# hherlyng/knp-emi-cgx

Measured on AMD Instinct MI355X. Metric: MDoF/s per implicit timestep (assembly+GMRES), higher is better.
Workload: dtype f64

## Files before the change

### knp-emi-cgx_amd/csrc/knp_internal.hpp

```cpp
#pragma once
#include <hip/hip_runtime.h>

#include <cstdint>
#include <string>
#include <vector>

#include "knpemi_hip.h"

#define KNP_NPROF 5

struct KnpHostGraph {
    int dim = 0, nv1 = 0;
    int n_v = 0, n_v_owned = 0, n_c = 0, n_c_owned = 0, n_g = 0, n_q = 0;
    int n_nodes = 0, n_nodes_owned = 0;
    std::vector<int32_t> node_i, node_e;
    std::vector<int32_t> node_vertex;
    std::vector<uint8_t> node_side;
    std::vector<int32_t> pair_ptr;
    std::vector<int32_t> pair_col;
    std::vector<int32_t> pair_row;
    std::vector<double> pair_M, pair_K;
    std::vector<int32_t> contrib_ptr;
    std::vector<int32_t> contrib_cell;
    std::vector<double> contrib_k;
// ... 163 lines not shown
    int l0_upload = 0;
    int32_t *at0_rp = nullptr, *at0_ci = nullptr;
    double* at0_v = nullptr;
    float* at0_vf = nullptr;
    int at0_lanes = 8;
    double *pt = nullptr, *pt_phi = nullptr;
    float *pt_f = nullptr, *pt_phi_f = nullptr;
};

struct KnpSidePrep {
    enum Kind { NONE, LEFT_ENQUEUED, LEFT_DEFERRED, LEFT_CONCURRENT, FLEX } kind = NONE;
    const double* b = nullptr;
    bool fused = false;
    bool left() const { return kind != NONE && kind != FLEX; }
};

struct knp_ctx {
    std::string err;
    hipStream_t stream = nullptr;
    int device = 0;
    KnpHostGraph g;
    double dt = 0, F = 1, C_M = 1, psi = 1;
    int n_ions = 3;
    double z[KNP_MAX_IONS] = {1, 1, -1}, Di[KNP_MAX_IONS] = {1, 1, 1}, De[KNP_MAX_IONS] = {1, 1, 1};
    int64_t nnz = 0, n_pairs = 0, n_contrib = 0, n_gp = 0, n_gc = 0;
    int n_dof_owned = 0, n_dof_local = 0;
    int32_t* d_cells = nullptr;
    uint8_t* d_cell_side = nullptr;
    double* d_coords = nullptr;
    int32_t* d_node_vertex = nullptr;
    uint8_t* d_node_side = nullptr;
    int32_t *d_node_i = nullptr, *d_node_e = nullptr;
    int32_t *d_pair_ptr = nullptr, *d_pair_col = nullptr, *d_pair_row = nullptr;
    double *d_pair_M = nullptr, *d_pair_K = nullptr;
    double2* d_pair_MK = nullptr;
    int32_t *d_contrib_ptr = nullptr, *d_contrib_cell = nullptr;
    double* d_contrib_k = nullptr;
    int32_t *d_node_cell_ptr = nullptr, *d_node_cell = nullptr;
    uint8_t* d_contrib_slot = nullptr;
    int64_t* d_tc_meta = nullptr;
    double* d_tc_k = nullptr;
    uint8_t* d_tc_slot = nullptr;
    int64_t n_tc = 0;
    int asm_stage = 0;
    int asm_dmax = 0;
    int64_t n_node_cells = 0;
    uint8_t* d_ncv = nullptr;
    double* d_knod = nullptr;
    int32_t* d_fv = nullptr;
    double* d_fmeas = nullptr;
    int32_t* d_gamma_prog = nullptr;
    double *d_qp = nullptr, *d_qw = nullptr;
    int32_t *d_gv_vertex = nullptr, *d_gv_node_i = nullptr, *d_gv_node_e = nullptr, *d_node_gv = nullptr;
    int32_t *d_gptr = nullptr, *d_gcol = nullptr, *d_grow = nullptr, *d_gq_i = nullptr, *d_gq_e = nullptr,
            *d_gdiag = nullptr;
    int32_t *d_gcptr = nullptr, *d_gc_facet = nullptr, *d_gc_lab = nullptr;
    double *d_at = nullptr, *d_ac = nullptr, *d_ax = nullptr;
    int32_t *d_gx_i = nullptr, *d_gx_e = nullptr;
    double* d_p_vals = nullptr;
    double* d_px = nullptr;
    int pc_coupled_phi = 0;
    bool have_A = false, have_P = false, have_cc = false;
    double* d_cbar = nullptr;
    double* d_fmat = nullptr;
    double* d_fvec = nullptr;
    std::vector<KnpProgram> progs;
    int32_t** d_prog_code = nullptr;
    double** d_prog_consts = nullptr;
    int32_t* d_prog_len = nullptr;
    int32_t* d_prog_nconsts = nullptr;
    int prog_regs = 0, prog_len_cap = 0, prog_consts_cap = 0;
    size_t gamma_lds_set = 0;
    void* jit_module = nullptr;
    void* jit_fn[3] = {nullptr, nullptr, nullptr};
    std::string jit_msg;
    bool progs_dirty = true;
    int max_prog = -1;
    const double* src_i[KNP_MAX_IONS] = {nullptr, nullptr, nullptr};
    const double* src_e[KNP_MAX_IONS] = {nullptr, nullptr, nullptr};
    bool have_sources = false;
    int pc_kind = KNP_PC_NONE;
    int fused_dots = 1;
    int spmv_dots = 1;
    double* d_vbj = nullptr;
    KnpAmgHier hier[KNP_MAX_HIER];
    int amg_fp32 = 0;
    float* d_p_vals_f = nullptr;
    double* d_ML = nullptr;
    double* d_cc = nullptr;
    double *d_t2 = nullptr, *d_w2 = nullptr;
    int ns_on = 0;
    int spmv_group = 8;
    int pc_group = 8;
    int asm_group = 8;
    int gm_restart = 0;
    double* d_V = nullptr;
    double *d_w = nullptr, *d_t = nullptr;
    double* d_Z = nullptr;
    int z_cap = 0;
    double* d_partial = nullptr;
    double* d_red = nullptr;
    double* h_red = nullptr;
    double* h_red_dev = nullptr;
    double* mirror() const { return (allreduce && p2p_red < 0) ? nullptr : h_red_dev; }
    int64_t phi_count_cached = -1;
    int64_t* h_seq = nullptr;
    int64_t* h_seq_dev = nullptr;
    int64_t seq_counter = 0;
    int asm_full = 0;
    double asm_dt = -1.0;
    int n_bc = 0;
    int32_t* d_bc_dofs = nullptr;
    int defl_m = 0;
    int32_t* d_defl_mode = nullptr;
    double* d_defl_einv = nullptr;
    double* d_y = nullptr;
    double* d_gm = nullptr;
    int gm_cap = 0;
    int64_t n_norm_fallback = 0;
    int n_red_blocks = 0;
    knp_halo_fn halo = nullptr;
    knp_allreduce_fn allreduce = nullptr;
    knp_level_comm_fn level_comm = nullptr;
    void* comm_user = nullptr;
    KnpP2P* p2p = nullptr;
    int p2p_fine = -1;
    int p2p_red = -1;
    bool hook_allreduce() const { return allreduce && p2p_red < 0; }
    int comm_rc = 0;
    int n_int = 0, n_bnd = 0;
    int32_t *d_nodes_int = nullptr, *d_nodes_bnd = nullptr;
    hipStream_t stream3 = nullptr;
    hipEvent_t ev_x = nullptr, ev_halo = nullptr;
    hipStream_t stream2 = nullptr;
    hipEvent_t ev_fork = nullptr, ev_join = nullptr;
    KnpSidePrep prep;
    bool side_ws = false;
    double *d_t2_s = nullptr, *d_w2_s = nullptr, *d_wb = nullptr, *d_partial_s = nullptr;
    hipStream_t stream_asm = nullptr;
    hipEvent_t ev_fork_asm = nullptr, ev_asm = nullptr;
    bool asm_pending = false;
    double last_bnorm = 0.0;
    int64_t n_allreduce = 0, n_halo = 0, n_readback = 0;
    int64_t n_fused_dots = 0;
    int64_t n_spmv_dots = 0;
    std::vector<hipEvent_t> tm_events;
    size_t tm_used = 0;
    KnpDiagMap diag_cells, diag_facets;
    KnpDiagMap diag_flux;
    double2* d_flux_rec = nullptr;
    KnpDiagMap diag_phim;
    int32_t* diag_code = nullptr;
    int diag_n_instr = 0, diag_n_regs = 0, diag_n_consts = 0;
    double diag_consts[KNP_DIAG_MAX_CONSTS] = {};
    bool diag_prog = false;
    KnpEmi emi;
    int prof_on = 0;
    std::vector<hipEvent_t> prof_pool;
    struct ProfRec { hipEvent_t a, b; int cls; };
    std::vector<ProfRec> prof_recs;
    double prof_ms[KNP_NPROF] = {0, 0, 0, 0, 0};
    int64_t prof_n[KNP_NPROF] = {0, 0, 0, 0, 0};
};

int knp_host_threads();
```

### knp-emi-cgx_amd/csrc/knp_kernels.hip

```cpp
#include <hip/hip_runtime.h>
#include <hip/hip_ext.h>

#include <algorithm>
#include <cmath>
#include <cstdio>
#include <cstdlib>
#include <cstring>
#include <new>

#include "knp_internal.hpp"

#define HIPCHK(call)                                                                       \
    do {                                                                                   \
        hipError_t e_ = (call);                                                            \
        if (e_ != hipSuccess) {                                                            \
            ctx->err = std::string(#call) + ": " + hipGetErrorString(e_);                  \
            return KNP_E_HIP;                                                              \
        }                                                                                  \
    } while (0)
#define KCHK(expr)                         \
    do {                                   \
        int rc_ = (expr);                  \
        if (rc_ != KNP_OK) return rc_;     \
    } while (0)
// ... 4163 lines not shown
            else launch_restrict_first_t<double>(st, L.R_lanes, nc, L.R_rp, Rci, L.R_v, L.r, C.b, cc, C.inv_diag, C.d, C.x);
            launch_spmv_mp<1>(st, C.A_lanes, C.n, C.A_rp, C.A_ci, C.A_v, C.A_vf, C.x, C.b, C.r);
        }
    }
    for (int l = H.cfused ? 0 : nl - 2; l >= 0; --l) {
        KnpAmgLevel& L = H.lv[l];
        KnpAmgLevel& C = H.lv[l + 1];
        const double c = cheb_c(L);
        const int n_act = L.S_n_act > 0 ? L.S_n_act : L.S_rows;
        const int32_t* rp = L.S_n_act > 0 ? L.S_act_rp : L.S_rp;
        if (l > 0) {
            if (L.S_vf) launch_level_up_t<float, 0>(st, L.S_lanes, n_act, L.S_n_act > 0 ? L.S_act_rows : nullptr, rp, L.S_ci, L.S_vf, C.x, L.inv_diag, L.b, L.r, L.x, c, c, L.x, nullptr);
            else launch_level_up_t<double, 0>(st, L.S_lanes, n_act, L.S_n_act > 0 ? L.S_act_rows : nullptr, rp, L.S_ci, L.S_v, C.x, L.inv_diag, L.b, L.r, L.x, c, c, L.x, nullptr);
        } else if (phi) {
            const int32_t* rows = L.S_n_act > 0 ? L.S_act_rows_c : nullptr;
            const double* ccp = ctx->pc_kind == KNP_PC_AMG_LT ? nullptr : ctx->d_cc;
            if (L.S_vf) launch_level_up_t<float, 1>(st, L.S_lanes, L.S_n_act > 0 ? n_act : nn, rows, rp, L.S_ci, L.S_vf, C.x, L.dinv_c, b, L.r, nullptr, c, c, z, ccp);
            else launch_level_up_t<double, 1>(st, L.S_lanes, L.S_n_act > 0 ? n_act : nn, rows, rp, L.S_ci, L.S_v, C.x, L.dinv_c, b, L.r, nullptr, c, c, z, ccp);
        } else {
            if (L.S_vf) launch_level_up_t<float, 0>(st, L.S_lanes, n_act, L.S_n_act > 0 ? L.S_act_rows : nullptr, rp, L.S_ci, L.S_vf, C.x, L.inv_diag, b, L.r, nullptr, c, c, z, nullptr);
            else launch_level_up_t<double, 0>(st, L.S_lanes, n_act, L.S_n_act > 0 ? L.S_act_rows : nullptr, rp, L.S_ci, L.S_v, C.x, L.inv_diag, b, L.r, nullptr, c, c, z, nullptr);
        }
    }
}

static int check_hier(knp_ctx* ctx, int h) {
    KnpAmgHier& H = ctx->hier[h];
    if (H.levels < 1 || H.lv[0].n != ctx->n_dof_owned) { ctx->err = "AMG hierarchy " + std::to_string(h) + " not supplied"; return KNP_E_STATE; }
    if (H.native0 == 0 && H.lv[0].A_nnz == 0 && H.levels > 1) {
        ctx->err = "AMG hierarchy " + std::to_string(h) + ": level 0 has no operator (uploaded for knp_amg_use_native_level0, which is off)";
        return KNP_E_STATE;
    }
    for (int l = 0; l < H.levels - 1; ++l) {
        const int expect = H.lv[l].repl_n > 0 ? H.lv[l + 1].n : H.lv[l + 1].n_loc;
        if (H.lv[l].n_coarse != expect) { ctx->err = "AMG level sizes inconsistent"; return KNP_E_STATE; }
        if (H.lv[l].repl_n > 0 && H.lv[l].repl_n != H.lv[l + 1].n) { ctx->err = "replicated coarse size mismatch"; return KNP_E_STATE; }
    }
    if (H.nc > 0 && H.nc != H.lv[H.levels - 1].n) { ctx->err = "AMG coarse inverse size mismatch"; return KNP_E_STATE; }
    return KNP_OK;
}

static int build_level_scaled(knp_ctx* ctx, int hidx, int l) {
    KnpAmgLevel& L = ctx->hier[hidx].lv[l];
    const double c = 1.0 / (0.5 * (1.1 + 0.1) * L.lambda_max);
    double* dloc = nullptr;
    HIPCHK(hipMalloc((void**)&dloc, (size_t)std::max(L.n_loc, 1) * sizeof(double)));
    HIPCHK(hipMemsetAsync(dloc, 0, (size_t)std::max(L.n_loc, 1) * sizeof(double), ctx->stream));
    HIPCHK(hipMemcpyAsync(dloc, L.inv_diag, (size_t)L.n * sizeof(double), hipMemcpyDeviceToDevice, ctx->stream));
    if (L.dist && level_comm_on(ctx)) level_exchange(ctx, hidx, l, 0, dloc);
    const int nblk = (int)std::min<int64_t>(nblocks(L.A_nnz), 8192);
    if (L.A_vf) {
        HIPCHK(hipMalloc((void**)&L.At_vf, (size_t)L.A_nnz * sizeof(float)));
        hipLaunchKernelGGL((k_build_at<float, float>), dim3(nblk), dim3(NT), 0, ctx->stream, L.A_nnz, L.A_ci, L.A_vf, dloc, c, L.At_vf);
    } else {
        HIPCHK(hipMalloc((void**)&L.At_v, (size_t)L.A_nnz * sizeof(double)));
        hipLaunchKernelGGL((k_build_at<double, double>), dim3(nblk), dim3(NT), 0, ctx->stream, L.A_nnz, L.A_ci, L.A_v, dloc, c, L.At_v);
    }
    HIPCHK(hipGetLastError());
    HIPCHK(hipStreamSynchronize(ctx->stream));
    (void)hipFree(dloc);
    if (ctx->comm_rc != KNP_OK) { const int rc = ctx->comm_rc; ctx->comm_rc = KNP_OK; return rc; }
    return KNP_OK;
}

int knp_pc_setup(knp_ctx* ctx, int32_t kind) {
    CHECK_CTX(ctx);
    side_discard(ctx);
    KCHK(join_asm(ctx));
    if (kind != KNP_PC_NONE && kind != KNP_PC_VBJACOBI && kind != KNP_PC_AMG && kind != KNP_PC_AMG_BT && kind != KNP_PC_AMG_LT) { ctx->err = "unknown pc kind"; return KNP_E_ARG; }
    if (kind == KNP_PC_AMG) KCHK(check_hier(ctx, 0));
    if (kind == KNP_PC_AMG_BT || kind == KNP_PC_AMG_LT) {
        KCHK(check_hier(ctx, 0));
        KCHK(check_hier(ctx, 1));
        if (!ctx->d_t2) {
            HIPCHK(hipMalloc((void**)&ctx->d_t2, std::max(ctx->n_dof_local, 1) * sizeof(double)));
            HIPCHK(hipMalloc((void**)&ctx->d_w2, std::max(ctx->n_dof_local, 1) * sizeof(double)));
            HIPCHK(hipMemset(ctx->d_t2, 0, std::max(ctx->n_dof_local, 1) * sizeof(double)));
            HIPCHK(hipMemset(ctx->d_w2, 0, std::max(ctx->n_dof_local, 1) * sizeof(double)));
        }
    }
    ctx->pc_kind = kind;
    ctx->fused_dots = !(getenv("KNP_FUSED_DOTS") && atoi(getenv("KNP_FUSED_DOTS")) == 0);
    ctx->spmv_dots = !(getenv("KNP_SPMV_DOTS") && atoi(getenv("KNP_SPMV_DOTS")) == 0);
    for (int h = 0; h < KNP_MAX_HIER; ++h) ctx->hier[h].fused = 0;
    if (kind == KNP_PC_AMG) ctx->hier[0].fused = fused_eligible(ctx, ctx->hier[0]) ? 1 : 0;
    if (kind == KNP_PC_AMG_BT || kind == KNP_PC_AMG_LT) {
        const bool ok = fused_eligible(ctx, ctx->hier[0]) && fused_eligible(ctx, ctx->hier[1]) && ctx->hier[1].native0 == 3 && ctx->hier[0].native0 == 2 &&
                        ctx->hier[1].lv[0].S_n_act > 0 && ctx->hier[1].lv[0].S_act_rows_c && ctx->hier[1].lv[0].R_ci_c;
        ctx->hier[0].fused = ctx->hier[1].fused = ok ? 1 : 0;
        if (!ok && ctx->hier[1].l0_upload) ctx->hier[1].native0 = 0;
    }
    for (int h = 0; h < KNP_MAX_HIER; ++h) {
        KnpAmgHier& H = ctx->hier[h];
        const bool off = getenv("KNP_BLOCKED") && atoi(getenv("KNP_BLOCKED")) == 0;
        bool ok = !off && H.fused && H.node_nf > 0 && (H.native0 == 1 || H.native0 == 2) && (H.native0 == 1) == (H.node_nf == 4);
        for (int l = 0; ok && l < H.levels - 1; ++l) {
            const KnpAmgLevel& L = H.lv[l];
            ok = L.bR.rp && L.bS.rp && (l == 0 || L.bA.rp) && L.bR.n_rows * H.node_nf == L.n_coarse &&
                 L.bS.n_rows * (l == 0 ? 4 : H.node_nf) == L.n;
        }
        H.blocked = ok ? 1 : 0;
        const bool coff = getenv("KNP_COARSE_FUSED") && atoi(getenv("KNP_COARSE_FUSED")) == 0;
        bool cok = !coff && H.fused && H.levels >= 3;
        for (int l = 1; cok && l < H.levels - 1; ++l) {
            const KnpAmgLevel& L = H.lv[l];
            cok = L.Rt_rp && L.U_rp && (!H.blocked || (L.bRt.rp && L.bU.rp && L.bRt.n_rows * H.node_nf == L.n_coarse && L.bU.n_rows * H.node_nf == L.n));
        }
        H.cfused = cok ? 1 : 0;
        for (int l = 1; cok && l < H.levels - 1; ++l) {
            KnpAmgLevel& L = H.lv[l];
            if (L.cat) continue;
            const size_t nc = (size_t)L.n + (size_t)L.n_coarse;
            HIPCHK(hipMalloc((void**)&L.cat, nc * sizeof(double)));
            HIPCHK(hipMemsetAsync(L.cat, 0, nc * sizeof(double), ctx->stream));
            ctx->side_ws = false;
        }
    }
    for (int h = 0; h < KNP_MAX_HIER; ++h) {
        KnpAmgHier& H = ctx->hier[h];
        const bool off = getenv("KNP_FUSED") && atoi(getenv("KNP_FUSED")) == 0;
        const KnpAmgLevel& L0 = H.lv[0];
        const bool have_pt = H.native0 == 3 ? (H.pt_phi || H.pt_phi_f) : (H.pt || H.pt_f);
        H.l0_fused = (!off && !H.fused && H.native0 > 0 && H.levels >= 2 && H.cheby == 1 && H.pre == 1 && H.post == 1 && L0.S_rp &&
                      L0.S_rows == L0.n && have_pt) ? 1 : 0;
        const bool used = (kind == KNP_PC_AMG && h == 0) || ((kind == KNP_PC_AMG_BT || kind == KNP_PC_AMG_LT) && h < 2);
        double veto[KNP_MAX_AMG_LEVELS] = {0};
        const bool lvl_off = getenv("KNP_FUSED_LEVELS") && atoi(getenv("KNP_FUSED_LEVELS")) == 0;
        for (int l = 1; l < H.levels - 1; ++l) {
            KnpAmgLevel& L = H.lv[l];
            dev_free(L.At_v); dev_free(L.At_vf);
            L.lfused = 0;
            const bool empty_here = L.dist && L.n == 0;
            const bool local_ok = !(!L.S_rp || L.S_rows != L.n || L.S_n_act > 0 || L.n_coarse <= 0 || L.A_nnz <= 0 || !L.inv_diag);
            veto[l] = (!used || off || lvl_off || H.fused || H.cheby != 1 || H.pre != 1 || H.post != 1 || !(local_ok || empty_here)) ? 1.0 : 0.0;
        }
        if (used && H.levels > 2) KCHK(global_sum_small(ctx, veto + 1, H.levels - 2));
        for (int l = 1; l < H.levels - 1; ++l) {
            if (veto[l] != 0.0) continue;
            KCHK(build_level_scaled(ctx, h, l));
            H.lv[l].lfused = 1;
        }
    }
    if (kind == KNP_PC_VBJACOBI && ctx->have_A) {
        const KnpHostGraph& g = ctx->g;
        hipLaunchKernelGGL(k_vbj_extract, dim3(nblocks(g.n_nodes_owned)), dim3(NT), 0, ctx->stream, g.n_nodes_owned,
                           ctx->d_pair_ptr, ctx->d_pair_col, ctx->d_ac, ctx->d_at, ctx->d_ax, ctx->d_node_gv, ctx->d_node_side,
                           ctx->d_gdiag, ctx->d_vbj);
        HIPCHK(hipGetLastError());
    }
    return KNP_OK;
}

__global__ void __launch_bounds__(NT) k_bc_copy(int n_bc, const int32_t* __restrict__ bc_dofs, const double* __restrict__ src,
                                                double* __restrict__ dst, int phi_only) {
    const int i = blockIdx.x * NT + threadIdx.x;
    if (i >= n_bc) return;
    const int d = bc_dofs[i];
    if (phi_only == 2) {
        if ((d & 3) == 3) dst[d >> 2] = src[d];
    } else if (!phi_only || (d & 3) == 3) {
        dst[d] = src[d];
    }
}

static int pc_apply_proj(knp_ctx* ctx, const double* r, double* z, int64_t cnt, DotReq* dq = nullptr) {
    const int dm = ctx->defl_m;
// ... 317 lines not shown
```

### knp-emi-cgx_amd/csrc/knp_krylov.inc

```

static constexpr int GM_RES = 100, GM_EXPL = 57, GM_MAX_RESTART = GM_EXPL - 2;
static constexpr int FB_SLOT = 124;
static_assert(GM_RES + 2 <= RED_SLOTS && DEFL_SLOT0 + DEFL_MAX <= GM_RES, "reduction slot layout");
static constexpr double GM_DTOL = 1e5;

static void side_discard(knp_ctx* ctx) {
    switch (ctx->prep.kind) {
        case KnpSidePrep::NONE:
        case KnpSidePrep::LEFT_DEFERRED: break;
        default: (void)hipEventSynchronize(ctx->ev_join);
    }
    ctx->prep.kind = KnpSidePrep::NONE;
}
static int ensure_side_stream(knp_ctx* ctx) {
    if (ctx->stream2) return KNP_OK;
    HIPCHK(hipStreamCreateWithFlags(&ctx->stream2, hipStreamNonBlocking));
    HIPCHK(hipEventCreateWithFlags(&ctx->ev_fork, hipEventDisableTiming));
    HIPCHK(hipEventCreateWithFlags(&ctx->ev_join, hipEventDisableTiming));
    return KNP_OK;
}

static bool exchanges_all_native(const knp_ctx* ctx) {
    if (!ctx->p2p || ctx->p2p_fine < 0 || ctx->p2p_red < 0 || ctx->defl_m > 0) return false;
    const int nh = ctx->pc_kind == KNP_PC_AMG ? 1 : (ctx->pc_kind == KNP_PC_AMG_BT || ctx->pc_kind == KNP_PC_AMG_LT) ? 2 : 0;
// ... 155 lines not shown
    ctx->z_cap = restart;
    return KNP_OK;
}

int knp_fgmres_prepare(knp_ctx* ctx, const double* b) {
    CHECK_CTX(ctx);
    if (!b) return KNP_E_ARG;
    side_discard(ctx);
    if (getenv("KNP_NO_PREPARE") || (ctx->prof_on & ~1) || ctx->halo || ctx->allreduce || ctx->level_comm || ctx->p2p) return KNP_OK;
    KCHK(ensure_side_stream(ctx));
    if (!ctx->d_partial_s) {
        HIPCHK(hipMalloc((void**)&ctx->d_partial_s, (size_t)RED_SLOTS * RED_BLOCKS * sizeof(double)));
        HIPCHK(hipMemset(ctx->d_partial_s, 0, (size_t)RED_SLOTS * RED_BLOCKS * sizeof(double)));
    }
    const int nb = ctx->n_red_blocks;
    HIPCHK(hipEventRecord(ctx->ev_fork, ctx->stream));
    HIPCHK(hipStreamWaitEvent(ctx->stream2, ctx->ev_fork, 0));
    hipLaunchKernelGGL(k_dot, dim3(nb), dim3(NT), 0, ctx->stream2, ctx->n_dof_owned, b, b, ctx->d_partial_s);
    hipLaunchKernelGGL(k_reduce_partials, dim3(1), dim3(NT), 0, ctx->stream2, nb, ctx->d_partial_s, ctx->d_red, FB_SLOT, ctx->mirror(),
                       (volatile int64_t*)nullptr, (int64_t)0);
    HIPCHK(hipGetLastError());
    HIPCHK(hipEventRecord(ctx->ev_join, ctx->stream2));
    ctx->prep = {KnpSidePrep::FLEX, b, false};
    return KNP_OK;
}

struct KrylovSolve {
    knp_ctx* ctx;
    GmLayout GL;
    double* gm;
    int n;
    int64_t ldv;
    int nb, vec_blocks;
    bool ns;
    double inv_cnt;
    double ttol, atol, dref;
};

static int krylov_begin(knp_ctx* ctx, const double* b, double* x, int32_t max_it, int32_t restart, int32_t* its, double* rnorm, int32_t* reason,
                        bool flexible, KrylovSolve* K, int64_t* cnt) {
    if (!b || !x || !its || !rnorm || !reason) return KNP_E_ARG;
    if (!ctx->have_A) { ctx->err = "matrix not assembled"; return KNP_E_STATE; }
    if (restart < 1 || restart > GM_MAX_RESTART || max_it < 0) {
        ctx->err = "restart must be in [1," + std::to_string(GM_MAX_RESTART) + "] and max_it >= 0";
        return KNP_E_ARG;
    }
    KCHK(ensure_work(ctx, restart));
    if (flexible && ctx->pc_kind != KNP_PC_NONE) KCHK(ensure_z(ctx, restart));
    prof_collect_ready(ctx);
    int rc;
    *cnt = ctx->ns_on ? global_phi_count(ctx, &rc) : 0;
    if (ctx->ns_on) KCHK(rc);
    const GmLayout GL{restart};
    if (ctx->gm_cap < GL.size()) {
        HIPCHK(hipStreamSynchronize(ctx->stream));
        dev_free(ctx->d_gm);
        HIPCHK(hipMalloc((void**)&ctx->d_gm, (size_t)GL.size() * sizeof(double)));
        HIPCHK(hipMemset(ctx->d_gm, 0, (size_t)GL.size() * sizeof(double)));
        ctx->gm_cap = GL.size();
    }
    const int n = ctx->n_dof_owned;
    *K = KrylovSolve{ctx, GL, ctx->d_gm, n, (int64_t)ctx->n_dof_local, ctx->n_red_blocks, std::min(nblocks(n), 2048), false, 0.0, 0.0, 0.0, 0.0};
    return KNP_OK;
}

static int gm_read_state(const KrylovSolve& K, double* res, int* flag) {
    knp_ctx* ctx = K.ctx;
    ++ctx->n_readback;
    if (ctx->mirror() && ctx->h_seq_dev) {
        KCHK(read_slots_inner(ctx, GM_RES, 2, ctx->seq_counter));
        if (ctx->p2p) KCHK(knp_p2p_check(ctx));
        *res = ctx->h_red[GM_RES];
        *flag = (int)ctx->h_red[GM_RES + 1];
    } else {
        double tmp[3];
        HIPCHK(hipMemcpyAsync(tmp, K.gm + K.GL.st(), 3 * sizeof(double), hipMemcpyDeviceToHost, ctx->stream));
        HIPCHK(hipStreamSynchronize(ctx->stream));
        *res = tmp[2];
        *flag = (int)tmp[1];
    }
    return KNP_OK;
}

static int arnoldi_step_finish(const KrylovSolve& K, int j, const double* w, double* vn, int first_nb, int first_stride, double* res, int* flag) {
    knp_ctx* ctx = K.ctx;
    hipStream_t st = ctx->stream;
    const GmLayout GL = K.GL;
    double* gm = K.gm;
    const int n = K.n, nb = K.nb, nsi = K.ns ? 1 : 0;
    const int64_t ldv = K.ldv;
    {
        ProfScope ps(ctx, 1);
        const bool done = first_nb > 0;
        const int nbr = done ? first_nb : nb;
        const int pst = done ? first_stride : RED_BLOCKS;
        for (int i0 = 0; i0 <= j && !done; i0 += 8) {
            if (i0 == 0 && K.ns)
                hipLaunchKernelGGL((k_multi_dot<8, true, true>), dim3(nb), dim3(NT), 0, st, n, ldv, i0, j + 1, ctx->d_V, w, ctx->d_partial);
            else if (i0 == 0)
                hipLaunchKernelGGL((k_multi_dot<8, false, true>), dim3(nb), dim3(NT), 0, st, n, ldv, i0, j + 1, ctx->d_V, w, ctx->d_partial);
            else
                hipLaunchKernelGGL((k_multi_dot<8, false, false>), dim3(nb), dim3(NT), 0, st, n, ldv, i0, j + 1, ctx->d_V, w, ctx->d_partial);
        }
        const int nred = j + 2 + nsi;
        if (fin_ok(ctx)) {
            ++ctx->n_allreduce;
            hipLaunchKernelGGL(k_reduce_fin, dim3(1), dim3(NT), 0, st, 1, nbr, nred, ctx->d_partial, ctx->d_red, 0, GL, j, nsi, K.inv_cnt, gm,
                               0, 0.0, ctx->mirror() ? ctx->h_red_dev + GM_RES : nullptr, ctx->mirror() ? ctx->h_seq_dev : nullptr, ++ctx->seq_counter,
                               pst);
        } else {
            hipLaunchKernelGGL(k_reduce_partials, dim3(nred), dim3(NT), 0, st, nbr, ctx->d_partial, ctx->d_red, 0, (double*)nullptr);
            KCHK(allreduce_slots(ctx, 0, nred));
            hipLaunchKernelGGL(k_givens, dim3(1), dim3(64), 0, st, GL, j, nsi, K.inv_cnt, ctx->d_red, -1, gm,
                               ctx->mirror() ? ctx->h_red_dev + GM_RES : nullptr, ctx->mirror() ? ctx->h_seq_dev : nullptr, ++ctx->seq_counter);
        }
        hipLaunchKernelGGL(k_update_scale, dim3(nb), dim3(NT), 0, st, n, ldv, j + 1, ctx->d_V, ctx->d_red, w, gm + GL.st(), K.inv_cnt, vn);
        HIPCHK(hipGetLastError());
    }
    KCHK(gm_read_state(K, res, flag));
    if (*flag == 1) {
        ProfScope ps(ctx, 1);
        ++ctx->n_norm_fallback;
        hipLaunchKernelGGL(k_dot, dim3(nb), dim3(NT), 0, st, n, vn, vn, ctx->d_partial);
        hipLaunchKernelGGL(k_reduce_partials, dim3(1), dim3(NT), 0, st, nb, ctx->d_partial, ctx->d_red, GM_EXPL, (double*)nullptr);
        KCHK(allreduce_slots(ctx, GM_EXPL, 1));
        hipLaunchKernelGGL(k_givens, dim3(1), dim3(64), 0, st, GL, j, nsi, K.inv_cnt, ctx->d_red, GM_EXPL, gm,
                           ctx->mirror() ? ctx->h_red_dev + GM_RES : nullptr, ctx->mirror() ? ctx->h_seq_dev : nullptr, ++ctx->seq_counter);
        hipLaunchKernelGGL(k_scale_inplace_rsqrt, dim3(K.vec_blocks), dim3(NT), 0, st, n, gm + GL.st(), vn);
        HIPCHK(hipGetLastError());
        KCHK(gm_read_state(K, res, flag));
    }
    return KNP_OK;
}

static bool krylov_stop_test(const KrylovSolve& K, int j, int flag, double res, int max_it, int* it, int* jd, int32_t* reason) {
    if (flag != 0 || !std::isfinite(res)) { *reason = KNP_DIVERGED_NANORINF; *jd = j; return true; }
    ++*it;
    *jd = j + 1;
    if (res <= K.ttol) { *reason = (res <= K.atol) ? KNP_CONVERGED_ATOL : KNP_CONVERGED_RTOL; return true; }
    if (*it >= max_it) { *reason = KNP_DIVERGED_ITS; return true; }
    if (res > GM_DTOL * K.dref) { *reason = KNP_DIVERGED_DTOL; return true; }
    return false;
}

static void krylov_update_plain(const KrylovSolve& K, int jd, const double* basis, double* x) {
    hipStream_t st = K.ctx->stream;
    if (jd <= 8) {
        hipLaunchKernelGGL(k_lincomb_solve, dim3(K.vec_blocks), dim3(NT), 0, st, K.GL, jd, K.gm, K.n, K.ldv, basis, x);
    } else {
        hipLaunchKernelGGL(k_gm_solve_y, dim3(1), dim3(64), 0, st, K.GL, jd, K.gm);
        hipLaunchKernelGGL(k_lincomb, dim3(K.vec_blocks), dim3(NT), 0, st, K.n, K.ldv, jd, basis, K.gm + K.GL.y(), x);
    }
}

static int krylov_end(const KrylovSolve& K, double* x, int it, double res, int32_t* its, double* rnorm) {
    knp_ctx* ctx = K.ctx;
    *its = it;
    *rnorm = res;
    KCHK(halo_update(ctx, x));
    HIPCHK(hipGetLastError());
    if (ctx->p2p) {
        HIPCHK(hipStreamSynchronize(ctx->stream));
        KCHK(knp_p2p_check(ctx));
    }
    if (ctx->comm_rc != KNP_OK) { const int rc2 = ctx->comm_rc; ctx->comm_rc = KNP_OK; return rc2; }
    return KNP_OK;
}

int knp_gmres_solve(knp_ctx* ctx, const double* b, double* x, double rtol, double atol, int32_t max_it, int32_t restart,
                    int32_t* its, double* rnorm, int32_t* reason) {
    CHECK_CTX(ctx);
    KrylovSolve K;
    int64_t cnt;
    KCHK(krylov_begin(ctx, b, x, max_it, restart, its, rnorm, reason, false, &K, &cnt));
    const int n = K.n, m = restart;
    const int64_t ldv = K.ldv;
    const GmLayout GL = K.GL;
    double* gm = K.gm;
    hipStream_t st = ctx->stream;

    bool lazy_bnorm = false;
    const bool prepared = ctx->prep.left() && ctx->prep.b == b && restart == ctx->gm_restart;
    if (prepared && ctx->prep.kind != KnpSidePrep::LEFT_ENQUEUED) {
        lazy_bnorm = true;
    } else if (prepared) {
        HIPCHK(hipEventSynchronize(ctx->ev_join));
        ctx->prep.kind = KnpSidePrep::NONE;
        if (!ctx->h_red_dev) {
            HIPCHK(hipMemcpy(ctx->h_red + 60, ctx->d_red + 60, 2 * sizeof(double), hipMemcpyDeviceToHost));
        }
        if (ctx->prep.fused && ctx->h_red[61] != 0.0) {
            ++ctx->n_norm_fallback;
            KCHK(pc_apply_proj(ctx, b, ctx->d_w, cnt));
            KCHK(dot_to_slot(ctx, ctx->d_w, ctx->d_w, 60));
            KCHK(read_slots(ctx, 60, 1, ctx->seq_counter));
        }
    } else {
        side_discard(ctx);
        bool fused_norm = false;
        KCHK(pc_apply_norm(ctx, b, ctx->d_w, cnt, &fused_norm));
        KCHK(pc_norm_read(ctx, ctx->d_w, cnt, &fused_norm));
    }
    double bnorm = lazy_bnorm ? 0.0 : std::sqrt(ctx->h_red[60]);
    ctx->last_bnorm = bnorm;
    if (!lazy_bnorm && !std::isfinite(bnorm)) { *its = 0; *rnorm = bnorm; *reason = KNP_DIVERGED_NANORINF; return KNP_OK; }
    K.ttol = std::max(rtol * bnorm, atol);
    K.atol = atol;
    int it = 0;
    double res = 0.0, res0 = -1.0;
    *reason = 0;
    const bool ns = ctx->ns_on && cnt > 0;
    K.ns = ns;
    K.inv_cnt = ns ? 1.0 / (double)cnt : 0.0;
    while (true) {
        KCHK(spmv_A(ctx, x, b, ctx->d_t, true));
        bool fused_norm = false;
        KCHK(pc_apply_norm(ctx, ctx->d_t, ctx->d_w, cnt, &fused_norm));
        if (lazy_bnorm && ctx->prep.kind == KnpSidePrep::LEFT_DEFERRED) {
            ctx->prep.kind = KnpSidePrep::LEFT_CONCURRENT;
            HIPCHK(hipStreamWaitEvent(ctx->stream2, ctx->ev_fork, 0));
            ctx->stream = ctx->stream2;
            bool fn = false;
            swap_side_ws(ctx);
            const int rcs = pc_apply_norm(ctx, b, ctx->d_wb, cnt, &fn, true);
            swap_side_ws(ctx);
            ctx->stream = st;
            KCHK(rcs);
            HIPCHK(hipEventRecord(ctx->ev_join, ctx->stream2));
        }
        KCHK(pc_norm_read(ctx, ctx->d_w, cnt, &fused_norm));
        if (lazy_bnorm) {
            lazy_bnorm = false;
            HIPCHK(hipEventSynchronize(ctx->ev_join));
            ctx->prep.kind = KnpSidePrep::NONE;
            double nb2 = ctx->h_red[SIDE_SLOT];
            if (ctx->h_red[SIDE_SLOT + 1] != 0.0) {
                ++ctx->n_norm_fallback;
                KCHK(pc_apply_proj(ctx, b, ctx->d_wb, cnt));
                KCHK(dot_to_slot(ctx, ctx->d_wb, ctx->d_wb, 60));
                KCHK(read_slots(ctx, 60, 1, ctx->seq_counter));
                nb2 = ctx->h_red[60];
                KCHK(pc_apply_norm(ctx, ctx->d_t, ctx->d_w, cnt, &fused_norm));
                KCHK(pc_norm_read(ctx, ctx->d_w, cnt, &fused_norm));
            }
            bnorm = std::sqrt(nb2);
            ctx->last_bnorm = bnorm;
            if (!std::isfinite(bnorm)) { *its = 0; *rnorm = bnorm; *reason = KNP_DIVERGED_NANORINF; return KNP_OK; }
            K.ttol = std::max(rtol * bnorm, atol);
        }
        const double beta = std::sqrt(ctx->h_red[60]);
        res = beta;
        if (res0 < 0) K.dref = res0 = beta;
        if (!std::isfinite(beta)) { *reason = KNP_DIVERGED_NANORINF; break; }
        if (beta <= K.ttol) { *reason = (beta <= atol) ? KNP_CONVERGED_ATOL : KNP_CONVERGED_RTOL; break; }
        if (it >= max_it) { *reason = KNP_DIVERGED_ITS; break; }
        if (fused_norm) {
            hipLaunchKernelGGL(k_scale_rsqrt_proj, dim3(K.vec_blocks), dim3(NT), 0, st, n, ctx->d_w, ctx->d_red + 60, ctx->d_red + 62,
                               1.0 / (double)cnt, ctx->d_V, gm + GL.g(), m);
        } else {
            hipLaunchKernelGGL(k_scale_rsqrt, dim3(K.vec_blocks), dim3(NT), 0, st, n, ctx->d_w, ctx->d_red + 60, ctx->d_V);
            hipLaunchKernelGGL(k_gm_init, dim3(1), dim3(64), 0, st, GL, gm, ctx->d_red + 60);
        }
        int jd = 0;
        bool stop = false;
        for (int j = 0; j < m; ++j) {
            double* vj = ctx->d_V + (size_t)j * ldv;
            double* vn = ctx->d_V + (size_t)(j + 1) * ldv;
            KCHK(spmv_A(ctx, vj, nullptr, ctx->d_t, false));
            DotReq dq{j + 1, ns, ldv, ctx->d_V, ctx->d_partial};
            KCHK(pc_apply_proj(ctx, ctx->d_t, ctx->d_w, ns ? 0 : cnt, (ctx->fused_dots && fin_ok(ctx) && j + 1 <= BU_MAX_M) ? &dq : nullptr));
            int flag = 0;
            KCHK(arnoldi_step_finish(K, j, ctx->d_w, vn, dq.done ? dq.nb : 0, RED_WIDE, &res, &flag));
            if (krylov_stop_test(K, j, flag, res, max_it, &it, &jd, reason)) { stop = true; break; }
        }
        if (jd > 0) {
            ProfScope ps(ctx, 1);
            krylov_update_plain(K, jd, ctx->d_V, x);
        }
        if (stop) break;
    }
    return krylov_end(K, x, it, res, its, rnorm);
}

int knp_fgmres_solve(knp_ctx* ctx, const double* b, double* x, double rtol, double atol, int32_t max_it, int32_t restart,
                     int32_t* its, double* rnorm, int32_t* reason) {
    CHECK_CTX(ctx);
    KrylovSolve K;
    int64_t cnt;
    KCHK(krylov_begin(ctx, b, x, max_it, restart, its, rnorm, reason, true, &K, &cnt));
    const bool pc_none = ctx->pc_kind == KNP_PC_NONE;
    const int n = K.n, nb = K.nb, m = restart;
    const int64_t ldv = K.ldv;
    const GmLayout GL = K.GL;
    double* gm = K.gm;
    hipStream_t st = ctx->stream;

    if (ctx->prep.kind == KnpSidePrep::FLEX && ctx->prep.b == b) {
        HIPCHK(hipEventSynchronize(ctx->ev_join));
        ctx->prep.kind = KnpSidePrep::NONE;
        if (!ctx->mirror()) HIPCHK(hipMemcpy(ctx->h_red + FB_SLOT, ctx->d_red + FB_SLOT, sizeof(double), hipMemcpyDeviceToHost));
    } else {
        side_discard(ctx);
        KCHK(dot_to_slot(ctx, b, b, FB_SLOT));
        KCHK(read_slots(ctx, FB_SLOT, 1, ctx->seq_counter));
    }
    const double bnorm = std::sqrt(ctx->h_red[FB_SLOT]);
    ctx->last_bnorm = bnorm;
    if (!std::isfinite(bnorm)) { *its = 0; *rnorm = bnorm; *reason = KNP_DIVERGED_NANORINF; return KNP_OK; }
    K.ttol = std::max(rtol * bnorm, atol);
    K.atol = atol;
    int it = 0;
    double res = 0.0, res0 = -1.0;
    *reason = 0;
    const bool ns = ctx->ns_on && cnt > 0;
    double* Zb = pc_none ? ctx->d_V : ctx->d_Z;
    while (true) {
        {
            int nbd = 0;
            if (launch_spmv_dots(ctx, x, b, ctx->d_w, 0, ldv, ctx->d_V, &nbd)) {
                ++ctx->n_allreduce;
                hipLaunchKernelGGL(k_reduce_fin, dim3(1), dim3(NT), 0, st, 3, nbd, 1, ctx->d_partial, ctx->d_red, 60, GL, 0, 0, 0.0, (double*)nullptr, 0,
                                   0.0, ctx->mirror(), ctx->mirror() ? ctx->h_seq_dev : nullptr, ++ctx->seq_counter, SPMV_WIDE);
                HIPCHK(hipGetLastError());
            } else {
                KCHK(spmv_A(ctx, x, b, ctx->d_w, true));
                KCHK(dot_to_slot(ctx, ctx->d_w, ctx->d_w, 60));
            }
            KCHK(read_slots(ctx, 60, 1, ctx->seq_counter));
        }
        const double beta = std::sqrt(ctx->h_red[60]);
        res = beta;
        if (res0 < 0) { res0 = beta; K.dref = bnorm > 0.0 ? bnorm : res0; }
        if (!std::isfinite(beta)) { *reason = KNP_DIVERGED_NANORINF; break; }
        if (beta <= K.ttol) { *reason = (beta <= atol) ? KNP_CONVERGED_ATOL : KNP_CONVERGED_RTOL; break; }
        if (it >= max_it) { *reason = KNP_DIVERGED_ITS; break; }
        hipLaunchKernelGGL(k_scale_rsqrt_proj, dim3(K.vec_blocks), dim3(NT), 0, st, n, ctx->d_w, ctx->d_red + 60, ctx->d_red + 60, 0.0, ctx->d_V,
                           gm + GL.g(), m);
        int jd = 0;
        bool stop = false;
        for (int j = 0; j < m; ++j) {
            double* vj = ctx->d_V + (size_t)j * ldv;
            double* vn = ctx->d_V + (size_t)(j + 1) * ldv;
            double* zj = Zb + (size_t)j * ldv;
            if (!pc_none) KCHK(pc_apply_proj(ctx, vj, zj, 0));
            int nbd = 0, flag = 0;
            const bool folded = j + 1 <= BU_MAX_M && launch_spmv_dots(ctx, zj, nullptr, ctx->d_w, j + 1, ldv, ctx->d_V, &nbd);
            if (!folded) KCHK(spmv_A(ctx, zj, nullptr, ctx->d_w, false));
            KCHK(arnoldi_step_finish(K, j, ctx->d_w, vn, folded ? nbd : 0, SPMV_WIDE, &res, &flag));
            if (krylov_stop_test(K, j, flag, res, max_it, &it, &jd, reason)) { stop = true; break; }
        }
        if (jd > 0) {
            ProfScope ps(ctx, 1);
            if (ns) {
                if (jd <= 8) {
                    hipLaunchKernelGGL(k_zcorr<true>, dim3(nb), dim3(NT), 0, st, GL, jd, gm, n, ldv, Zb, ctx->d_t, ctx->d_partial);
// ... 17 lines not shown
```

Baseline: 2165.

## Speculatively enqueue first GMRES Arnoldi step before reading initial residual norm

In the GMRES restart loop, the change enqueues the v0 normalization and the first Arnoldi iteration (SpMV, preconditioner, dots, Givens) before reading back the initial residual norm. The host then waits once for both the norm and the first step's state instead of synchronizing twice. This removes one host-device round trip per restart cycle in single-device runs. If the fused norm signals a fallback, the residual is recomputed and the speculative work is discarded. That costs extra work on those cycles and also when the initial residual is already converged.

```diff
diff --git a/knp-emi-cgx_amd/csrc/knp_internal.hpp b/knp-emi-cgx_amd/csrc/knp_internal.hpp
--- a/knp-emi-cgx_amd/csrc/knp_internal.hpp
+++ b/knp-emi-cgx_amd/csrc/knp_internal.hpp
@@ -269,6 +269,7 @@
     int pc_kind = KNP_PC_NONE;
     int fused_dots = 1;
     int spmv_dots = 1;
+    int gmres_ahead = 1;
     double* d_vbj = nullptr;
     KnpAmgHier hier[KNP_MAX_HIER];
     int amg_fp32 = 0;
diff --git a/knp-emi-cgx_amd/csrc/knp_kernels.hip b/knp-emi-cgx_amd/csrc/knp_kernels.hip
--- a/knp-emi-cgx_amd/csrc/knp_kernels.hip
+++ b/knp-emi-cgx_amd/csrc/knp_kernels.hip
@@ -4269,6 +4269,7 @@
     ctx->pc_kind = kind;
     ctx->fused_dots = !(getenv("KNP_FUSED_DOTS") && atoi(getenv("KNP_FUSED_DOTS")) == 0);
     ctx->spmv_dots = !(getenv("KNP_SPMV_DOTS") && atoi(getenv("KNP_SPMV_DOTS")) == 0);
+    ctx->gmres_ahead = !(getenv("KNP_GMRES_AHEAD") && atoi(getenv("KNP_GMRES_AHEAD")) == 0);
     for (int h = 0; h < KNP_MAX_HIER; ++h) ctx->hier[h].fused = 0;
     if (kind == KNP_PC_AMG) ctx->hier[0].fused = fused_eligible(ctx, ctx->hier[0]) ? 1 : 0;
     if (kind == KNP_PC_AMG_BT || kind == KNP_PC_AMG_LT) {
diff --git a/knp-emi-cgx_amd/csrc/knp_krylov.inc b/knp-emi-cgx_amd/csrc/knp_krylov.inc
--- a/knp-emi-cgx_amd/csrc/knp_krylov.inc
+++ b/knp-emi-cgx_amd/csrc/knp_krylov.inc
@@ -261,42 +261,48 @@
     return KNP_OK;
 }
 
-static int arnoldi_step_finish(const KrylovSolve& K, int j, const double* w, double* vn, int first_nb, int first_stride, double* res, int* flag) {
+static int arnoldi_step_enqueue(const KrylovSolve& K, int j, const double* w, double* vn, int first_nb, int first_stride) {
     knp_ctx* ctx = K.ctx;
     hipStream_t st = ctx->stream;
     const GmLayout GL = K.GL;
     double* gm = K.gm;
     const int n = K.n, nb = K.nb, nsi = K.ns ? 1 : 0;
     const int64_t ldv = K.ldv;
-    {
-        ProfScope ps(ctx, 1);
-        const bool done = first_nb > 0;
-        const int nbr = done ? first_nb : nb;
-        const int pst = done ? first_stride : RED_BLOCKS;
-        for (int i0 = 0; i0 <= j && !done; i0 += 8) {
-            if (i0 == 0 && K.ns)
-                hipLaunchKernelGGL((k_multi_dot<8, true, true>), dim3(nb), dim3(NT), 0, st, n, ldv, i0, j + 1, ctx->d_V, w, ctx->d_partial);
-            else if (i0 == 0)
-                hipLaunchKernelGGL((k_multi_dot<8, false, true>), dim3(nb), dim3(NT), 0, st, n, ldv, i0, j + 1, ctx->d_V, w, ctx->d_partial);
-            else
-                hipLaunchKernelGGL((k_multi_dot<8, false, false>), dim3(nb), dim3(NT), 0, st, n, ldv, i0, j + 1, ctx->d_V, w, ctx->d_partial);
-        }
-        const int nred = j + 2 + nsi;
-        if (fin_ok(ctx)) {
-            ++ctx->n_allreduce;
-            hipLaunchKernelGGL(k_reduce_fin, dim3(1), dim3(NT), 0, st, 1, nbr, nred, ctx->d_partial, ctx->d_red, 0, GL, j, nsi, K.inv_cnt, gm,
-                               0, 0.0, ctx->mirror() ? ctx->h_red_dev + GM_RES : nullptr, ctx->mirror() ? ctx->h_seq_dev : nullptr, ++ctx->seq_counter,
-                               pst);
-        } else {
-            hipLaunchKernelGGL(k_reduce_partials, dim3(nred), dim3(NT), 0, st, nbr, ctx->d_partial, ctx->d_red, 0, (double*)nullptr);
-            KCHK(allreduce_slots(ctx, 0, nred));
-            hipLaunchKernelGGL(k_givens, dim3(1), dim3(64), 0, st, GL, j, nsi, K.inv_cnt, ctx->d_red, -1, gm,
-                               ctx->mirror() ? ctx->h_red_dev + GM_RES : nullptr, ctx->mirror() ? ctx->h_seq_dev : nullptr, ++ctx->seq_counter);
-        }
-        hipLaunchKernelGGL(k_update_scale, dim3(nb), dim3(NT), 0, st, n, ldv, j + 1, ctx->d_V, ctx->d_red, w, gm + GL.st(), K.inv_cnt, vn);
-        HIPCHK(hipGetLastError());
-    }
-    KCHK(gm_read_state(K, res, flag));
+    ProfScope ps(ctx, 1);
+    const bool done = first_nb > 0;
+    const int nbr = done ? first_nb : nb;
+    const int pst = done ? first_stride : RED_BLOCKS;
+    for (int i0 = 0; i0 <= j && !done; i0 += 8) {
+        if (i0 == 0 && K.ns)
+            hipLaunchKernelGGL((k_multi_dot<8, true, true>), dim3(nb), dim3(NT), 0, st, n, ldv, i0, j + 1, ctx->d_V, w, ctx->d_partial);
+        else if (i0 == 0)
+            hipLaunchKernelGGL((k_multi_dot<8, false, true>), dim3(nb), dim3(NT), 0, st, n, ldv, i0, j + 1, ctx->d_V, w, ctx->d_partial);
+        else
+            hipLaunchKernelGGL((k_multi_dot<8, false, false>), dim3(nb), dim3(NT), 0, st, n, ldv, i0, j + 1, ctx->d_V, w, ctx->d_partial);
+    }
+    const int nred = j + 2 + nsi;
+    if (fin_ok(ctx)) {
+        ++ctx->n_allreduce;
+        hipLaunchKernelGGL(k_reduce_fin, dim3(1), dim3(NT), 0, st, 1, nbr, nred, ctx->d_partial, ctx->d_red, 0, GL, j, nsi, K.inv_cnt, gm,
+                           0, 0.0, ctx->mirror() ? ctx->h_red_dev + GM_RES : nullptr, ctx->mirror() ? ctx->h_seq_dev : nullptr, ++ctx->seq_counter,
+                           pst);
+    } else {
+        hipLaunchKernelGGL(k_reduce_partials, dim3(nred), dim3(NT), 0, st, nbr, ctx->d_partial, ctx->d_red, 0, (double*)nullptr);
+        KCHK(allreduce_slots(ctx, 0, nred));
+        hipLaunchKernelGGL(k_givens, dim3(1), dim3(64), 0, st, GL, j, nsi, K.inv_cnt, ctx->d_red, -1, gm,
+                           ctx->mirror() ? ctx->h_red_dev + GM_RES : nullptr, ctx->mirror() ? ctx->h_seq_dev : nullptr, ++ctx->seq_counter);
+    }
+    hipLaunchKernelGGL(k_update_scale, dim3(nb), dim3(NT), 0, st, n, ldv, j + 1, ctx->d_V, ctx->d_red, w, gm + GL.st(), K.inv_cnt, vn);
+    HIPCHK(hipGetLastError());
+    return KNP_OK;
+}
+static int arnoldi_step_read(const KrylovSolve& K, int j, double* vn, double* res, int* flag, bool have = false) {
+    knp_ctx* ctx = K.ctx;
+    hipStream_t st = ctx->stream;
+    const GmLayout GL = K.GL;
+    double* gm = K.gm;
+    const int n = K.n, nb = K.nb, nsi = K.ns ? 1 : 0;
+    if (!have) KCHK(gm_read_state(K, res, flag));
     if (*flag == 1) {
         ProfScope ps(ctx, 1);
         ++ctx->n_norm_fallback;
@@ -311,6 +317,10 @@
     }
     return KNP_OK;
 }
+static int arnoldi_step_finish(const KrylovSolve& K, int j, const double* w, double* vn, int first_nb, int first_stride, double* res, int* flag) {
+    KCHK(arnoldi_step_enqueue(K, j, w, vn, first_nb, first_stride));
+    return arnoldi_step_read(K, j, vn, res, flag);
+}
 
 static bool krylov_stop_test(const KrylovSolve& K, int j, int flag, double res, int max_it, int* it, int* jd, int32_t* reason) {
     if (flag != 0 || !std::isfinite(res)) { *reason = KNP_DIVERGED_NANORINF; *jd = j; return true; }
@@ -391,6 +401,25 @@
     const bool ns = ctx->ns_on && cnt > 0;
     K.ns = ns;
     K.inv_cnt = ns ? 1.0 / (double)cnt : 0.0;
+    auto enqueue_v0 = [&](bool fused_norm) {
+        if (fused_norm) {
+            hipLaunchKernelGGL(k_scale_rsqrt_proj, dim3(K.vec_blocks), dim3(NT), 0, st, n, ctx->d_w, ctx->d_red + 60, ctx->d_red + 62,
+                               1.0 / (double)cnt, ctx->d_V, gm + GL.g(), m);
+        } else {
+            hipLaunchKernelGGL(k_scale_rsqrt, dim3(K.vec_blocks), dim3(NT), 0, st, n, ctx->d_w, ctx->d_red + 60, ctx->d_V);
+            hipLaunchKernelGGL(k_gm_init, dim3(1), dim3(64), 0, st, GL, gm, ctx->d_red + 60);
+        }
+    };
+    auto enqueue_iteration = [&](int j) -> int {
+        double* vj = ctx->d_V + (size_t)j * ldv;
+        double* vn = ctx->d_V + (size_t)(j + 1) * ldv;
+        KCHK(spmv_A(ctx, vj, nullptr, ctx->d_t, false));
+        DotReq dq{j + 1, ns, ldv, ctx->d_V, ctx->d_partial};
+        KCHK(pc_apply_proj(ctx, ctx->d_t, ctx->d_w, ns ? 0 : cnt, (ctx->fused_dots && fin_ok(ctx) && j + 1 <= BU_MAX_M) ? &dq : nullptr));
+        return arnoldi_step_enqueue(K, j, ctx->d_w, vn, dq.done ? dq.nb : 0, RED_WIDE);
+    };
+    const bool ahead_ok = ctx->gmres_ahead && ctx->mirror() && ctx->h_seq && ctx->h_seq_dev && !ctx->halo && !ctx->allreduce && !ctx->p2p &&
+                          !ctx->level_comm && ctx->defl_m == 0 && ctx->n_bc == 0 && max_it > 0 && (ctx->prof_on & ~1) == 0;
     while (true) {
         KCHK(spmv_A(ctx, x, b, ctx->d_t, true));
         bool fused_norm = false;
@@ -407,7 +436,23 @@
             KCHK(rcs);
             HIPCHK(hipEventRecord(ctx->ev_join, ctx->stream2));
         }
-        KCHK(pc_norm_read(ctx, ctx->d_w, cnt, &fused_norm));
+        bool ahead = ahead_ok && fused_norm;
+        double res_a = 0.0;
+        int flag_a = 0;
+        auto redo_residual = [&]() -> int {
+            if (ahead) KCHK(spmv_A(ctx, x, b, ctx->d_t, true));
+            ahead = false;
+            KCHK(pc_apply_norm(ctx, ctx->d_t, ctx->d_w, cnt, &fused_norm));
+            return pc_norm_read(ctx, ctx->d_w, cnt, &fused_norm);
+        };
+        if (ahead) {
+            enqueue_v0(true);
+            KCHK(enqueue_iteration(0));
+            KCHK(gm_read_state(K, &res_a, &flag_a));
+            if (ctx->h_red[61] != 0.0) KCHK(redo_residual());
+        } else {
+            KCHK(pc_norm_read(ctx, ctx->d_w, cnt, &fused_norm));
+        }
         if (lazy_bnorm) {
             lazy_bnorm = false;
             HIPCHK(hipEventSynchronize(ctx->ev_join));
@@ -419,8 +464,7 @@
                 KCHK(dot_to_slot(ctx, ctx->d_wb, ctx->d_wb, 60));
                 KCHK(read_slots(ctx, 60, 1, ctx->seq_counter));
                 nb2 = ctx->h_red[60];
-                KCHK(pc_apply_norm(ctx, ctx->d_t, ctx->d_w, cnt, &fused_norm));
-                KCHK(pc_norm_read(ctx, ctx->d_w, cnt, &fused_norm));
+                KCHK(redo_residual());
             }
             bnorm = std::sqrt(nb2);
             ctx->last_bnorm = bnorm;
@@ -433,23 +477,15 @@
         if (!std::isfinite(beta)) { *reason = KNP_DIVERGED_NANORINF; break; }
         if (beta <= K.ttol) { *reason = (beta <= atol) ? KNP_CONVERGED_ATOL : KNP_CONVERGED_RTOL; break; }
         if (it >= max_it) { *reason = KNP_DIVERGED_ITS; break; }
-        if (fused_norm) {
-            hipLaunchKernelGGL(k_scale_rsqrt_proj, dim3(K.vec_blocks), dim3(NT), 0, st, n, ctx->d_w, ctx->d_red + 60, ctx->d_red + 62,
-                               1.0 / (double)cnt, ctx->d_V, gm + GL.g(), m);
-        } else {
-            hipLaunchKernelGGL(k_scale_rsqrt, dim3(K.vec_blocks), dim3(NT), 0, st, n, ctx->d_w, ctx->d_red + 60, ctx->d_V);
-            hipLaunchKernelGGL(k_gm_init, dim3(1), dim3(64), 0, st, GL, gm, ctx->d_red + 60);
-        }
+        if (!ahead) enqueue_v0(fused_norm);
         int jd = 0;
         bool stop = false;
         for (int j = 0; j < m; ++j) {
-            double* vj = ctx->d_V + (size_t)j * ldv;
-            double* vn = ctx->d_V + (size_t)(j + 1) * ldv;
-            KCHK(spmv_A(ctx, vj, nullptr, ctx->d_t, false));
-            DotReq dq{j + 1, ns, ldv, ctx->d_V, ctx->d_partial};
-            KCHK(pc_apply_proj(ctx, ctx->d_t, ctx->d_w, ns ? 0 : cnt, (ctx->fused_dots && fin_ok(ctx) && j + 1 <= BU_MAX_M) ? &dq : nullptr));
-            int flag = 0;
-            KCHK(arnoldi_step_finish(K, j, ctx->d_w, vn, dq.done ? dq.nb : 0, RED_WIDE, &res, &flag));
+            const bool have = ahead && j == 0;
+            int flag = have ? flag_a : 0;
+            if (have) res = res_a;
+            else KCHK(enqueue_iteration(j));
+            KCHK(arnoldi_step_read(K, j, ctx->d_V + (size_t)(j + 1) * ldv, &res, &flag, have));
             if (krylov_stop_test(K, j, flag, res, max_it, &it, &jd, reason)) { stop = true; break; }
         }
         if (jd > 0) {
```

After: 2207 (median of 6 runs). 1.02x the previous value.
